# sephiroce/srf

Measured on AMD Instinct MI355X. Metric: acoustic frames/sec through SRF (123-d fbank, 3-iter DR) at 1/2/4/8 MI355X, higher is better.
Workload: dtype fp32; 1 GPU; wsj_c4: SRF L=6 PH=CH=16 DIM=32 LPAD=RPAD=2 DR iter=3, train step (fwd+bwd+allreduce+Adam); utterances_per_gpu=28, frames_per_utterance=800, global_batch=28, parallelism=dp1, launch=hipgraph (fwd+CTC+bwd)

## Files before the change

### srf_amd/csrc/cnnfe.hip

```cpp
#include <algorithm>
#include <type_traits>
#include <cmath>
#include <cstdlib>

#include "srf_common.h"
#include "srf_reduce.h"
#include "srf_rng.h"
#include "../../include/srf.h"

namespace {

constexpr int C = 64;
constexpr float kBnEps = 1e-3f;
constexpr float kBnMomentum = 0.99f;

struct Dims {
  int B, T, Fin;
  int T1, F1, T2, F2;
  int pt1, pf1, pt2, pf2;
};

inline int same_out(int n) { return (n + 1) / 2; }
inline int same_pad_before(int n) {
  const int out = same_out(n);
// ... 784 lines not shown
      return;
    } else {
    cbf8 a1, a2, a3;
    {
      float v[8];
#pragma unroll
      for (int q = 0; q < 8; ++q) v[q] = aok ? (q < 4 ? av[0][q] : av[1][q - 4]) : 0.f;
      split8v(v, a1, a2, a3);
    }
#pragma unroll
    for (int nt = 0; nt < 2; ++nt) {
      const int nrow = 32 * nt + r;
      const cbf8 b1 = *reinterpret_cast<const cbf8*>(&Bs[buf][0][nrow * kC2BStride + 8 * h]);
      const cbf8 b2 = *reinterpret_cast<const cbf8*>(&Bs[buf][1][nrow * kC2BStride + 8 * h]);
      const cbf8 b3 = *reinterpret_cast<const cbf8*>(&Bs[buf][2][nrow * kC2BStride + 8 * h]);
      cf16 cc = acc[nt];
      cc = mfma32bf(a3, b1, cc);
      cc = mfma32bf(a1, b3, cc);
      cc = mfma32bf(a2, b2, cc);
      cc = mfma32bf(a2, b1, cc);
      cc = mfma32bf(a1, b2, cc);
      cc = mfma32bf(a1, b1, cc);
      acc[nt] = cc;
    }
    }
  };
  V8 bvA[NBL], bvB[NBL];
  f4 avA[2], avB[2];
  bool okA, okB;
  load_b(0, bvA);
  load_a(0, avA, okA);
  load_b(1, bvB);
  load_a(1, avB, okB);
  store_b(0, bvA);
  __syncthreads();
  for (int kk = 0; kk < nkb; kk += 2) {
    {
      const f4 a0[2] = {avA[0], avA[1]};
      const bool ok0 = okA;
      if (kk + 2 < nkb) {
        load_b(kk + 2, bvA);
        load_a(kk + 2, avA, okA);
      }
      compute(0, a0, ok0);
      store_b(1, bvB);
      __syncthreads();
    }
    {
      const f4 a1v[2] = {avB[0], avB[1]};
      const bool ok1 = okB;
      if (kk + 3 < nkb) {
        load_b(kk + 3, bvB);
        load_a(kk + 3, avB, okB);
      }
      compute(1, a1v, ok1);
      if (kk + 2 < nkb) store_b(0, bvA);
      __syncthreads();
    }
  }
  float osc[2] = {1.f, 1.f};
  if constexpr (H) {
    osc[0] = inv_sa * wdsc[r];
    osc[1] = inv_sa * wdsc[32 + r];
  }
#pragma unroll
  for (int q = 0; q < 4; ++q)
#pragma unroll
    for (int v = 0; v < 4; ++v) {
      const int p = q0 + 32 * wv + 8 * q + 4 * h + v;
      if (p >= Pc) continue;
      const int kf = p % nkf, kt = (p / nkf) % nkt, b = p / (nkf * nkt);
      float* dst = g_x1 + (((size_t)b * d.T1 + qt + 2 * kt) * d.F1 + qf + 2 * kf) * C + r;
      dst[0] = H ? acc[0][4 * q + v] * osc[0] : acc[0][4 * q + v];
      dst[32] = H ? acc[1][4 * q + v] * osc[1] : acc[1][4 * q + v];
    }
}

constexpr int kWgChunk = 32;

struct WgDiv {
  FastDiv f2, t2;
};

constexpr int kTpPx = 64;
template <bool H>
__global__ __launch_bounds__(256) void gab_split_t_kernel(const float* __restrict__ g_ab, int P2, int P2p,
                                                          void* __restrict__ gsTv, const float* __restrict__ gmax,
                                                          int ngmax) {
  __shared__ float tile[kTpPx][2 * C + 1];
  const int tid = threadIdx.x;
  const int p0 = blockIdx.x * kTpPx;
  float sa = 1.f;
  if constexpr (H) sa = srf_exp2i(gab_exp(gmax, ngmax));
  for (int k = tid; k < kTpPx * (2 * C / 4); k += 256) {
    const int px = k / (2 * C / 4), q = k % (2 * C / 4);
    const int p = p0 + px;
    const f4 v = p < P2 ? *reinterpret_cast<const f4*>(g_ab + (size_t)p * 2 * C + 4 * q) : f4{0.f, 0.f, 0.f, 0.f};
    tile[px][4 * q] = v.x;
    tile[px][4 * q + 1] = v.y;
    tile[px][4 * q + 2] = v.z;
    tile[px][4 * q + 3] = v.w;
  }
  __syncthreads();
  const size_t plane = (size_t)2 * C * P2p;
  for (int task = tid; task < 2 * C * (kTpPx / 8); task += 256) {
    const int o = task & 7, n = task >> 3;
    float v[8];
#pragma unroll
    for (int k = 0; k < 8; ++k) v[k] = tile[8 * o + k][n];
    if constexpr (H) {
      ch8 p1, p2;
#pragma unroll
      for (int k = 0; k < 8; ++k) {
        _Float16 h1, h2;
        srf_split2h(v[k] * sa, h1, h2);
        p1[k] = h1;
        p2[k] = h2;
      }
      _Float16* dst = static_cast<_Float16*>(gsTv) + (size_t)n * P2p + p0 + 8 * o;
      *reinterpret_cast<ch8*>(dst) = p1;
      *reinterpret_cast<ch8*>(dst + plane) = p2;
    } else {
      cbf8 p1, p2, p3;
      split8v(v, p1, p2, p3);
      __bf16* dst = static_cast<__bf16*>(gsTv) + (size_t)n * P2p + p0 + 8 * o;
      *reinterpret_cast<cbf8*>(dst) = p1;
      *reinterpret_cast<cbf8*>(dst + plane) = p2;
      *reinterpret_cast<cbf8*>(dst + 2 * plane) = p3;
    }
  }
}

constexpr int kW2Chunk = 32;
constexpr int kW2AStride = 96;

typedef short ws4 __attribute__((ext_vector_type(4)));

template <typename BT>
__device__ __forceinline__ ws4 lds_tr16(const BT* p) {
  return __builtin_amdgcn_ds_read_tr16_b64_v4i16(
      (__attribute__((address_space(3))) ws4*)(reinterpret_cast<uintptr_t>(p)));
}

template <bool H>
__global__ __launch_bounds__(256) __attribute__((amdgpu_waves_per_eu(2))) void conv2_wgrad32_kernel(
    const float* __restrict__ y1, const float* __restrict__ stats1, const int* __restrict__ inp_len,
    const void* __restrict__ gsTv, int P2p, Dims d, WgDiv dv, int nsplit, int split_len, float* __restrict__ part,
    const float* __restrict__ gmax, int ngmax) {
  using BT = std::conditional_t<H, _Float16, __bf16>;
  using V8 = std::conditional_t<H, ch8, cbf8>;
  constexpr int NPL = H ? 2 : 3;
  const BT* __restrict__ gsT3 = static_cast<const BT*>(gsTv);
  __shared__ __attribute__((aligned(16))) BT As[2][NPL][kW2Chunk * kW2AStride];
  float out_sc = 1.f;
  if constexpr (H) out_sc = stats1[4 * C + 1] * srf_exp2i(-gab_exp(gmax, ngmax));
  const int tid = threadIdx.x, lane = tid & 63, wv = tid >> 6;
  const int r = lane & 31, h = lane >> 5;
  const int xcd = blockIdx.x & 7, loc = blockIdx.x >> 3;
  const int tap = loc % 9, sp = xcd + 8 * (loc / 9);
  const int dt = tap / 3, df = tap - dt * 3;
  const int P2 = d.B * d.T2 * d.F2;
  const int pbeg = sp * split_len, pend = min(P2, pbeg + split_len);
  const int px = tid >> 3, oc = tid & 7;
  float scale[8], shift[8];
  const float bsc = H ? stats1[4 * C] : 1.f;
#pragma unroll
  for (int k = 0; k < 8; ++k) {
    scale[k] = stats1[2 * C + 8 * oc + k] * bsc;
    shift[k] = stats1[3 * C + 8 * oc + k] * bsc;
  }
  f4 xv[2];
  bool xok = false;
  auto gather = [&](int pc0) {
    const int p = pc0 + px;
    const unsigned pcl = (unsigned)min(p, P2 - 1);
    const unsigned r1 = fdiv(pcl, dv.f2);
    const int f2 = (int)(pcl - r1 * d.F2);
    const unsigned bq = fdiv(r1, dv.t2);
    const int t2 = (int)(r1 - bq * d.T2), b = (int)bq;
    const int t1 = 2 * t2 - d.pt2 + dt, f1 = 2 * f2 - d.pf2 + df;
    xok = p < pend && t1 >= 0 && t1 < d.T1 && f1 >= 0 && f1 < d.F1 && t1 < ceil_div_len(inp_len[b], 2);
    const int t1c = min(max(t1, 0), d.T1 - 1), f1c = min(max(f1, 0), d.F1 - 1);
    const float* src = y1 + (((size_t)b * d.T1 + t1c) * d.F1 + f1c) * C + 8 * oc;
    xv[0] = *reinterpret_cast<const f4*>(src);
    xv[1] = *reinterpret_cast<const f4*>(src + 4);
  };
  auto put = [&](int buf) {
    float v[8];
#pragma unroll
    for (int k = 0; k < 8; ++k) v[k] = xok ? (k < 4 ? xv[0][k] : xv[1][k - 4]) * scale[k] + shift[k] : 0.f;
    const int o = px * kW2AStride + 8 * oc;
    if constexpr (H) {
      ch8 p1, p2;
#pragma unroll
      for (int k = 0; k < 8; ++k) {
        _Float16 h1, h2;
        srf_split2h(v[k], h1, h2);
        p1[k] = h1;
        p2[k] = h2;
      }
      *reinterpret_cast<ch8*>(&As[buf][0][o]) = p1;
      *reinterpret_cast<ch8*>(&As[buf][1][o]) = p2;
    } else {
      cbf8 p1, p2, p3;
      split8v(v, p1, p2, p3);
      *reinterpret_cast<cbf8*>(&As[buf][0][o]) = p1;
      *reinterpret_cast<cbf8*>(&As[buf][1][o]) = p2;
      *reinterpret_cast<cbf8*>(&As[buf][2][o]) = p3;
    }
  };
  const int gg = lane >> 4, qq = (lane >> 2) & 3, pp = lane & 3;
  const int a_off = (8 * (gg >> 1) + qq) * kW2AStride + 16 * (gg & 1) + 4 * pp;
  auto read_a = [&](const BT* img, int kb, int mt) {
    const BT* base = img + a_off + 16 * kb * kW2AStride + 32 * mt;
    const ws4 lo = lds_tr16(base), hi = lds_tr16(base + 4 * kW2AStride);
    return __builtin_bit_cast(V8, __builtin_shufflevector(lo, hi, 0, 1, 2, 3, 4, 5, 6, 7));
  };
  const size_t bplane = (size_t)2 * C * P2p;
  const BT* brow = gsT3 + (size_t)(32 * wv + r) * P2p + 8 * h;
  V8 bc[2][NPL], bn[2][NPL];
  auto load_bf = [&](int pc0, V8 (&bf)[2][NPL]) {
#pragma unroll
    for (int kb = 0; kb < 2; ++kb)
#pragma unroll
      for (int pl = 0; pl < NPL; ++pl) bf[kb][pl] = *reinterpret_cast<const V8*>(brow + pl * bplane + pc0 + 16 * kb);
  };

  cf16 acc[2];
  acc[0] = cf16{};
  acc[1] = cf16{};
  const int nch = (pend - pbeg + kW2Chunk - 1) / kW2Chunk;
  if (nch > 0) {
    gather(pbeg);
    load_bf(pbeg, bc);
    put(0);
  }
  __syncthreads();
  for (int ch = 0; ch < nch; ++ch) {
    const bool more = ch + 1 < nch;
    const int buf = ch & 1;
    if (more) {
      gather(pbeg + (ch + 1) * kW2Chunk);
      load_bf(pbeg + (ch + 1) * kW2Chunk, bn);
    }
#pragma unroll
    for (int kb = 0; kb < 2; ++kb)
#pragma unroll
      for (int mt = 0; mt < 2; ++mt) {
        if constexpr (H) {
          const ch8 a1 = read_a(As[buf][0], kb, mt);
          const ch8 a2 = read_a(As[buf][1], kb, mt);
          cf16 cc = acc[mt];
          cc = mfma32h(a2, bc[kb][0], cc);
          cc = mfma32h(a1, bc[kb][1], cc);
          cc = mfma32h(a1, bc[kb][0], cc);
          acc[mt] = cc;
        } else {
          const cbf8 a1 = read_a(As[buf][0], kb, mt);
          const cbf8 a2 = read_a(As[buf][1], kb, mt);
          const cbf8 a3 = read_a(As[buf][2], kb, mt);
          cf16 cc = acc[mt];
          cc = mfma32bf(a3, bc[kb][0], cc);
          cc = mfma32bf(a1, bc[kb][2], cc);
          cc = mfma32bf(a2, bc[kb][1], cc);
          cc = mfma32bf(a2, bc[kb][0], cc);
          cc = mfma32bf(a1, bc[kb][1], cc);
          cc = mfma32bf(a1, bc[kb][0], cc);
          acc[mt] = cc;
        }
      }
    if (more) {
      put(buf ^ 1);
#pragma unroll
      for (int kb = 0; kb < 2; ++kb)
#pragma unroll
        for (int pl = 0; pl < NPL; ++pl) bc[kb][pl] = bn[kb][pl];
    }
    __syncthreads();
  }
  float* dst = part + ((size_t)sp * 9 + tap) * C * 2 * C + 32 * wv + r;
#pragma unroll
  for (int mt = 0; mt < 2; ++mt)
#pragma unroll
    for (int q = 0; q < 4; ++q)
#pragma unroll
      for (int v = 0; v < 4; ++v) dst[(size_t)(32 * mt + 8 * q + 4 * h + v) * 2 * C] = acc[mt][4 * q + v] * out_sc;
}

__global__ void conv2_wgrad_reduce_kernel(const float* __restrict__ part, int nsplit, float* __restrict__ gka,
                                          float* __restrict__ gkb) {
  const int idx = blockIdx.x * blockDim.x + threadIdx.x;
  if (idx >= 9 * C * 2 * C) return;
  float s = 0.f;
#pragma unroll 8
  for (int k = 0; k < nsplit; ++k) s += part[(size_t)k * 9 * C * 2 * C + idx];
  const int n = idx % (2 * C);
  const int tc = idx / (2 * C);
  if (n < C)
    gka[(size_t)tc * C + n] = s;
  else
    gkb[(size_t)tc * C + n - C] = s;
}

__global__ __launch_bounds__(256) void conv1_bwd_kernel(
    const float* __restrict__ feats, const int* __restrict__ inp_len, Dims d, const float* __restrict__ g_x1,
    const float* __restrict__ y1, const unsigned char* __restrict__ sel1, const float* __restrict__ stats1,
    const float* __restrict__ gamma1, const float* __restrict__ bnsum1, float drop_p, unsigned long long seed, const unsigned long long* __restrict__ seed_src,
    float* __restrict__ part) {
  seed = srf_step_seed(seed, seed_src);
  extern __shared__ __attribute__((aligned(16))) float win[];
  __shared__ float sh[kRows1][20][C];
  const int c = threadIdx.x & (C - 1);
  const int w = __builtin_amdgcn_readfirstlane(threadIdx.x >> 6);
  const int P = d.B * d.T1 * d.F1;
  const float mean = stats1[c], rstd = stats1[C + c], gam = gamma1[c];
  const float sdy_n = bnsum1[c] / (float)P, sdyxh_n = bnsum1[C + c] / (float)P;
  const float keep_scale = 1.f / (1.f - drop_p);
  float acc[20];
#pragma unroll
  for (int j = 0; j < 20; ++j) acc[j] = 0.f;
  const Tile1 tl = stage_rows1(feats, d, win);
  const int t1 = tl.t1_0 + w;
  if (t1 < d.T1) {
    const float mask = t1 < ceil_div_len(inp_len[tl.b], 2) ? 1.f : 0.f;
    const int pbase = (tl.b * d.T1 + t1) * d.F1;
    constexpr int FB = 8;
    for (int f0 = 0; f0 < d.F1; f0 += FB) {
      float gxv[FB], yv[FB];
      unsigned char sv[FB];
#pragma unroll
      for (int u = 0; u < FB; ++u) {
        const int o = (pbase + min(f0 + u, d.F1 - 1)) * C + c;
        gxv[u] = g_x1[o];
        yv[u] = y1[o];
        sv[u] = sel1[o];
      }
#pragma unroll
      for (int u = 0; u < FB; ++u) {
        const int f1 = f0 + u;
        if (f1 >= d.F1) break;
        const int o = (pbase + f1) * C + c;
        const float gy = bn_bwd_elem(gxv[u], yv[u], mask, mean, rstd, gam, sdy_n, sdyxh_n);
        const bool sl = sv[u] != 0;
        float ga = sl ? gy : 0.f, gb = sl ? 0.f : gy;
        if (drop_p > 0.f) {
          bool ka, kb;
          srf_keep2(seed, kStreamConv0a, o, drop_p, ka, kb);
          ga *= ka ? keep_scale : 0.f;
          gb *= kb ? keep_scale : 0.f;
        }
        float x[9];
        window9_lds(win, tl, d, w, f1, x);
        acc[18] += ga;
        acc[19] += gb;
#pragma unroll
        for (int k = 0; k < 9; ++k) {
          acc[k] += x[k] * ga;
          acc[9 + k] += x[k] * gb;
        }
      }
    }
  }
#pragma unroll
  for (int j = 0; j < 20; ++j) sh[w][j][c] = acc[j];
  __syncthreads();
  for (int j = w; j < 20; j += kRows1) {
    float v = 0.f;
#pragma unroll
    for (int r = 0; r < kRows1; ++r) v += sh[r][j][c];
    part[((size_t)blockIdx.x * 20 + j) * C + c] = v;
  }
}

inline int conv1_blocks(const Dims& d) { return d.B * ((d.T1 + kRows1 - 1) / kRows1); }
inline size_t conv1_lds(const Dims& d) { return (size_t)(2 * kRows1 + 1) * (d.Fin + 2) * sizeof(float); }

struct FwdSaved {
  float *y1, *y2, *stats1, *stats2;
  unsigned char *sel1, *sel2;
  size_t bytes;
};

FwdSaved saved_layout(const Dims& d, void* base) {
  const size_t P1 = (size_t)d.B * d.T1 * d.F1, P2 = (size_t)d.B * d.T2 * d.F2;
  size_t off = 0;
  auto take = [&](size_t bytes) {
    size_t o = off;
    off += srf::align_up(bytes, 256);
    return o;
  };
  const size_t oy1 = take(P1 * C * 4), oy2 = take(P2 * C * 4), os1 = take(5 * C * 4), os2 = take(5 * C * 4),
               osel1 = take(P1 * C), osel2 = take(P2 * C);
  char* b = static_cast<char*>(base);
  FwdSaved s;
  s.y1 = (float*)(b + oy1);
  s.y2 = (float*)(b + oy2);
  s.stats1 = (float*)(b + os1);
  s.stats2 = (float*)(b + os2);
  s.sel1 = (unsigned char*)(b + osel1);
  s.sel2 = (unsigned char*)(b + osel2);
  s.bytes = off;
  return s;
}

constexpr int kBnMerge = 32;

int bn_finalize(const float* part, int nparts, float* merged, const float* gamma, const float* beta, float* mmean,
                float* mvar, int training, float* stats, hipStream_t st, const float* ymax = nullptr,
                int nymax = 0) {
  const int per = (nparts + kBnMerge - 1) / kBnMerge;
  hipLaunchKernelGGL(bn_merge_kernel, dim3(kBnMerge), dim3(256), 0, st, part, nparts, per, merged);
  SRF_LAUNCH_CHECK("bn_merge");
  hipLaunchKernelGGL(bn_finalize_kernel, dim3(1), dim3(1024), 0, st, merged, kBnMerge, gamma, beta, mmean, mvar,
                     training, stats, ymax, nymax);
  SRF_LAUNCH_CHECK("bn_finalize");
  return SRF_OK;
}

struct FwdWs {
  float *part1, *part2, *wp, *merged;
  _Float16* wp2;
  float* wsc;
  float* ymax;
  size_t bytes;
};

FwdWs fwd_ws_layout(const Dims& d, void* base) {
  const size_t P2 = (size_t)d.B * d.T2 * d.F2;
  const size_t nb2 = (P2 + 63) / 64;
  size_t off = 0;
  auto take = [&](size_t bytes) {
    size_t o = off;
    off += srf::align_up(bytes, 256);
    return o;
  };
  const size_t op1 = take((size_t)conv1_blocks(d) * 3 * C * 4), op2 = take(nb2 * 3 * C * 4),
               owp = take((size_t)9 * 2 * C * C * 4), omg = take((size_t)kBnMerge * 3 * C * 4),
               owp2 = take((size_t)2 * 9 * 2 * C * C * 2), owsc = take((size_t)2 * C * 4),
               oym = take((size_t)conv1_blocks(d) * 4);
  char* b = static_cast<char*>(base);
  FwdWs w;
  w.wp2 = (_Float16*)(b + owp2);
  w.wsc = (float*)(b + owsc);
  w.ymax = (float*)(b + oym);
  w.merged = (float*)(b + omg);
  w.part1 = (float*)(b + op1);
  w.part2 = (float*)(b + op2);
  w.wp = (float*)(b + owp);
  w.bytes = off;
  return w;
}

int check_dims(int B, int T, int Fin, int nfilt) {
  SRF_REQUIRE(B > 0 && T > 0 && Fin > 0, "bad CNN-FE shape B=%d T=%d F=%d", B, T, Fin);
  SRF_REQUIRE(nfilt == C, "model-conv-filter-num must be %d (got %d)", C, nfilt);
  return SRF_OK;
}

}

extern "C" {

int srf_cnnfe_out_dims(int T, int feat_dim, int* T2, int* F2) {
  SRF_REQUIRE(T > 0 && feat_dim > 0 && T2 && F2, "bad arguments");
  Dims d = make_dims(1, T, feat_dim);
  *T2 = d.T2;
  *F2 = d.F2;
  return SRF_OK;
}

size_t srf_cnnfe_saved_bytes(int B, int T, int feat_dim, int nfilt) {
  (void)nfilt;
  return saved_layout(make_dims(B, T, feat_dim), nullptr).bytes;
}

size_t srf_cnnfe_fwd_workspace(int B, int T, int feat_dim, int nfilt) {
  (void)nfilt;
  return fwd_ws_layout(make_dims(B, T, feat_dim), nullptr).bytes;
}

int srf_cnnfe_fwd(const float* feats, const int* inp_len, int B, int T, int feat_dim, int nfilt,
                  const float* k0a, const float* b0a, const float* k0b, const float* b0b, const float* gamma0,
                  const float* beta0, const float* k1a, const float* b1a, const float* k1b, const float* b1b,
                  const float* gamma1, const float* beta1, float* mmean0, float* mvar0, float* mmean1, float* mvar1,
                  int training, float drop_p, unsigned long long seed, float* out, void* saved, size_t saved_bytes,
                  void* workspace, size_t workspace_bytes, void* stream) {
  int rc = check_dims(B, T, feat_dim, nfilt);
  if (rc) return rc;
  SRF_REQUIRE(feats && inp_len && k0a && b0a && k0b && b0b && gamma0 && beta0 && k1a && b1a && k1b && b1b &&
                  gamma1 && beta1 && mmean0 && mvar0 && mmean1 && mvar1 && out && saved && workspace,
              "null pointer argument");
  SRF_REQUIRE(drop_p >= 0.f && drop_p < 1.f, "dropout rate %f out of [0,1)", drop_p);
  const Dims d = make_dims(B, T, feat_dim);
  FwdSaved sv = saved_layout(d, saved);
  FwdWs w = fwd_ws_layout(d, workspace);
  if (saved_bytes < sv.bytes || workspace_bytes < w.bytes) {
    srf::set_error("CNN-FE buffers too small (saved %zu < %zu or workspace %zu < %zu)", saved_bytes, sv.bytes,
                   workspace_bytes, w.bytes);
    return SRF_EWORKSPACE;
  }
  hipStream_t st = static_cast<hipStream_t>(stream);
  const size_t P2 = (size_t)d.B * d.T2 * d.F2;
  const int nb2 = (int)((P2 + 63) / 64);
  int nparts2 = nb2;
  const int npack = (kPackW2Threads + 64 * kRows1 - 1) / (64 * kRows1);
  hipLaunchKernelGGL(conv1_fwd_kernel, dim3(conv1_blocks(d) + npack), dim3(64 * kRows1), conv1_lds(d), st, feats,
                     inp_len, d, k0a, b0a, k0b, b0b, training, drop_p, seed, srf::seed_source(), sv.y1, sv.sel1,
                     w.part1, conv1_blocks(d), k1a, k1b, w.wp2, w.wsc, w.ymax);
  SRF_LAUNCH_CHECK("conv1_fwd");
  if ((rc = bn_finalize(w.part1, conv1_blocks(d), w.merged, gamma0, beta0, mmean0, mvar0, training, sv.stats1, st,
                        w.ymax, conv1_blocks(d))))
    return rc;
  SRF_LAUNCH_CHECK("bn_finalize(1)");
  {
    const int nb32 = (int)((P2 + kC2Px - 1) / kC2Px);
    hipLaunchKernelGGL(conv2_fwd32_kernel, dim3(nb32), dim3(64 * kC2Waves), 0, st, sv.y1, sv.stats1, inp_len, d,
                       w.wp2, w.wsc, b1a, b1b, training, drop_p, seed, srf::seed_source(), sv.y2, sv.sel2,
                       w.part2);
    SRF_LAUNCH_CHECK("conv2_fwd32");
    nparts2 = nb32;
  }
  if ((rc = bn_finalize(w.part2, nparts2, w.merged, gamma1, beta1, mmean1, mvar1, training, sv.stats2, st)))
    return rc;
  SRF_LAUNCH_CHECK("bn_finalize(2)");
  hipLaunchKernelGGL(bn_apply_kernel, dim3(1024), dim3(256), 0, st, sv.y2, sv.stats2, inp_len, d.B, d.T2, d.F2, 4,
                     out);
  SRF_LAUNCH_CHECK("bn_apply");
  return SRF_OK;
}

}

namespace {
struct BwdWs2 {
  float *bnpart, *bnsum2, *bnsum1, *g_ab, *biaspart, *g_x1, *wq, *wpart, *c1part, *c1sum, *scratch;
  __bf16* gsT3;
  float* gmax;
  float* wdsc;
  int P2p;
  size_t bytes;
};

constexpr int kBnBlocks = 1024;
constexpr int kWgrad32SplitsMax = 128;
constexpr int kWgrad32Splits = 56;

BwdWs2 bwd_ws_layout(const Dims& d, void* base) {
  const size_t P1 = (size_t)d.B * d.T1 * d.F1, P2 = (size_t)d.B * d.T2 * d.F2;
  size_t off = 0;
  auto take = [&](size_t bytes) {
    size_t o = off;
    off += srf::align_up(bytes, 256);
    return o;
  };
  const size_t obp = take((size_t)kBnBlocks * 2 * C * 4), os2 = take(2 * C * 4), os1 = take(2 * C * 4),
               oab = take(P2 * 2 * C * 4), obias = take((size_t)kBnBlocks * 2 * C * 4), ogx = take(P1 * C * 4),
               owq = take((size_t)9 * 2 * C * C * 4), owp = take((size_t)kWgrad32SplitsMax * 9 * C * 2 * C * 4),
               oc1 = take((size_t)conv1_blocks(d) * 20 * C * 4), oc1s = take(20 * C * 4),
               oscr = take(srf::colsum_scratch_floats(std::max(conv1_blocks(d), kBnBlocks), 20 * C) * 4);
  const int P2p = (int)((P2 + kTpPx - 1) / kTpPx * kTpPx);
  const size_t ogs3 = take((size_t)3 * 2 * C * P2p * 2);
  const size_t ogm = take((size_t)kBnBlocks * 4), ods = take((size_t)C * 4);
  char* b = static_cast<char*>(base);
  BwdWs2 w;
  w.bnpart = (float*)(b + obp);
  w.bnsum2 = (float*)(b + os2);
  w.bnsum1 = (float*)(b + os1);
  w.g_ab = (float*)(b + oab);
  w.biaspart = (float*)(b + obias);
  w.g_x1 = (float*)(b + ogx);
  w.wq = (float*)(b + owq);
  w.wpart = (float*)(b + owp);
  w.c1part = (float*)(b + oc1);
  w.c1sum = (float*)(b + oc1s);
  w.scratch = (float*)(b + oscr);
  w.gsT3 = (__bf16*)(b + ogs3);
  w.gmax = (float*)(b + ogm);
  w.wdsc = (float*)(b + ods);
  w.P2p = P2p;
  w.bytes = off;
  return w;
}

}

extern "C" {

size_t srf_cnnfe_bwd_workspace(int B, int T, int feat_dim, int nfilt) {
  (void)nfilt;
  return bwd_ws_layout(make_dims(B, T, feat_dim), nullptr).bytes;
}

int srf_cnnfe_bwd(const float* feats, const int* inp_len, int B, int T, int feat_dim, int nfilt, const float* gamma0,
                  const float* k1a, const float* k1b, const float* gamma1, float drop_p, unsigned long long seed,
                  const void* saved, const float* g_out, float* g_k0a, float* g_b0a, float* g_k0b, float* g_b0b,
                  float* g_gamma0, float* g_beta0, float* g_k1a, float* g_b1a, float* g_k1b, float* g_b1b,
                  float* g_gamma1, float* g_beta1, void* workspace, size_t workspace_bytes, void* stream) {
  return srf_cnnfe_bwd_parts(SRF_CNNFE_BWD_ALL, feats, inp_len, B, T, feat_dim, nfilt, gamma0, k1a, k1b, gamma1, drop_p,
                             seed, saved, g_out, g_k0a, g_b0a, g_k0b, g_b0b, g_gamma0, g_beta0, g_k1a, g_b1a, g_k1b,
                             g_b1b, g_gamma1, g_beta1, workspace, workspace_bytes, stream);
}

int srf_cnnfe_bwd_parts(int parts, const float* feats, const int* inp_len, int B, int T, int feat_dim, int nfilt,
                        const float* gamma0, const float* k1a, const float* k1b, const float* gamma1, float drop_p,
                        unsigned long long seed, const void* saved, const float* g_out, float* g_k0a, float* g_b0a,
                        float* g_k0b, float* g_b0b, float* g_gamma0, float* g_beta0, float* g_k1a, float* g_b1a,
                        float* g_k1b, float* g_b1b, float* g_gamma1, float* g_beta1, void* workspace,
                        size_t workspace_bytes, void* stream) {
  SRF_REQUIRE(parts > 0 && (parts & ~SRF_CNNFE_BWD_ALL) == 0, "CNN-FE backward: bad parts mask %d", parts);
  int rc = check_dims(B, T, feat_dim, nfilt);
  if (rc) return rc;
  SRF_REQUIRE(feats && inp_len && gamma0 && k1a && k1b && gamma1 && saved && g_out && g_k0a && g_b0a && g_k0b &&
                  g_b0b && g_gamma0 && g_beta0 && g_k1a && g_b1a && g_k1b && g_b1b && g_gamma1 && g_beta1 &&
                  workspace,
              "null pointer argument");
  SRF_REQUIRE(((uintptr_t)g_out & 15) == 0 && ((uintptr_t)saved & 255) == 0 && ((uintptr_t)workspace & 255) == 0,
              "CNN-FE backward: g_out must be 16-byte and saved / workspace 256-byte aligned");
  const Dims d = make_dims(B, T, feat_dim);
  FwdSaved sv = saved_layout(d, const_cast<void*>(saved));
  BwdWs2 w = bwd_ws_layout(d, workspace);
  if (workspace_bytes < w.bytes) {
    srf::set_error("CNN-FE backward workspace too small: %zu < %zu", workspace_bytes, w.bytes);
    return SRF_EWORKSPACE;
  }
  hipStream_t st = static_cast<hipStream_t>(stream);
  const int P2 = d.B * d.T2 * d.F2;
  __bf16* wq3 = reinterpret_cast<__bf16*>(w.wq);
  _Float16* wq2h = reinterpret_cast<_Float16*>(w.wq);
  if (parts & SRF_CNNFE_BWD_PREP) {
  hipLaunchKernelGGL(bn_bwd_reduce_kernel, dim3(kBnBlocks), dim3(256), 0, st, g_out, sv.y2, sv.stats2, inp_len, d.B,
                     d.T2, d.F2, 4, w.bnpart);
  SRF_LAUNCH_CHECK("bn_bwd_reduce(2)");
  if ((rc = srf::colsum(w.bnpart, kBnBlocks, 2 * C, w.bnsum2, w.scratch, st, srf::ColSplit{{g_beta1, g_gamma1, nullptr, nullptr}, {C, C, 0, 0}})))
    return rc;
  const int npack = (kPackW2tF16Threads + 255) / 256;
  hipLaunchKernelGGL(conv2_bwd_prep_kernel, dim3(kBnBlocks + npack), dim3(256), 0, st, g_out, sv.y2, sv.sel2,
                     sv.stats2, gamma1, w.bnsum2, inp_len, d, drop_p, seed, srf::seed_source(), w.g_ab, w.biaspart,
                     kBnBlocks, k1a, k1b, wq3, wq2h, w.wdsc, w.gmax);
  SRF_LAUNCH_CHECK("conv2_bwd_prep");
  if ((rc = srf::colsum(w.biaspart, kBnBlocks, 2 * C, nullptr, w.scratch, st, srf::ColSplit{{g_b1a, g_b1b, nullptr, nullptr}, {C, C, 0, 0}})))
    return rc;
  }
  if (parts & SRF_CNNFE_BWD_DATA) {
    DgCls cls{};
    for (int c = 0; c < 4; ++c) {
      const int qt = c >> 1, qf = c & 1;
      const int Pc = d.B * ((d.T1 - qt + 1) / 2) * ((d.F1 - qf + 1) / 2);
      cls.boff[c + 1] = cls.boff[c] + (Pc + kD2Px - 1) / kD2Px;
    }
    hipLaunchKernelGGL(conv2_dgrad32_kernel<true>, dim3(cls.boff[4]), dim3(64 * kD2Waves), 0, st, w.g_ab,
                       (const void*)wq2h, d, cls, w.g_x1, (const float*)w.gmax, kBnBlocks, (const float*)w.wdsc);
    SRF_LAUNCH_CHECK("conv2_dgrad32");
  }
  const WgDiv dv{make_fastdiv(d.F2), make_fastdiv(d.T2)};
  const int nsplit = kWgrad32Splits;
  if (parts & SRF_CNNFE_BWD_WGRAD) {
    static_assert(kW2Chunk == kWgChunk, "wgrad splits are whole chunks");
    const int split_len = ((P2 + nsplit - 1) / nsplit + kWgChunk - 1) / kWgChunk * kWgChunk;
    hipLaunchKernelGGL(gab_split_t_kernel<true>, dim3(w.P2p / kTpPx), dim3(256), 0, st, w.g_ab, P2, w.P2p,
                       (void*)w.gsT3, (const float*)w.gmax, kBnBlocks);
    SRF_LAUNCH_CHECK("gab_split_t");
    hipLaunchKernelGGL(conv2_wgrad32_kernel<true>, dim3(9 * nsplit), dim3(256), 0, st, sv.y1, sv.stats1, inp_len,
                       (const void*)w.gsT3, w.P2p, d, dv, nsplit, split_len, w.wpart, (const float*)w.gmax,
                       kBnBlocks);
    SRF_LAUNCH_CHECK("conv2_wgrad32");
    hipLaunchKernelGGL(conv2_wgrad_reduce_kernel, dim3((9 * C * 2 * C + 255) / 256), dim3(256), 0, st, w.wpart,
                       nsplit, g_k1a, g_k1b);
    SRF_LAUNCH_CHECK("conv2_wgrad_reduce");
  }
  if (!(parts & SRF_CNNFE_BWD_DATA)) return SRF_OK;
  hipLaunchKernelGGL(bn_bwd_reduce_kernel, dim3(kBnBlocks), dim3(256), 0, st, w.g_x1, sv.y1, sv.stats1, inp_len, d.B,
                     d.T1, d.F1, 2, w.bnpart);
  SRF_LAUNCH_CHECK("bn_bwd_reduce(1)");
  if ((rc = srf::colsum(w.bnpart, kBnBlocks, 2 * C, w.bnsum1, w.scratch, st, srf::ColSplit{{g_beta0, g_gamma0, nullptr, nullptr}, {C, C, 0, 0}})))
    return rc;
  hipLaunchKernelGGL(conv1_bwd_kernel, dim3(conv1_blocks(d)), dim3(64 * kRows1), conv1_lds(d), st, feats, inp_len, d, w.g_x1, sv.y1,
                     sv.sel1, sv.stats1, gamma0, w.bnsum1, drop_p, seed, srf::seed_source(), w.c1part);
  SRF_LAUNCH_CHECK("conv1_bwd");
  if ((rc = srf::colsum(w.c1part, conv1_blocks(d), 20 * C, nullptr, w.scratch, st,
                        srf::ColSplit{{g_k0a, g_k0b, g_b0a, g_b0b, nullptr, nullptr}, {9 * C, 9 * C, C, C, 0, 0}})))
    return rc;
  return SRF_OK;
}

}
```

Before: 3.035 million frames/s.

## Compute conv2 weight gradient by time rows with fused fp16-split staging

Adds a row-range conv2 weight-gradient kernel for F2<=32. Each block streams output time rows, normalises y1 and scales g_ab in registers, splits them into fp16 hi/lo pairs in LDS, and runs three MFMAs per tap. The input rows are kept in a four-slot ring so the overlapping time tap is reused. This removes the separate gab_split_t transpose pass and its bf16 workspace. The trade-off is 256 partial slabs, which need a wider reduction kernel and more workspace, and a different fp16-split precision path.

```diff
diff --git a/srf_amd/csrc/cnnfe.hip b/srf_amd/csrc/cnnfe.hip
--- a/srf_amd/csrc/cnnfe.hip
+++ b/srf_amd/csrc/cnnfe.hip
@@ -1110,6 +1110,186 @@
     gkb[(size_t)tc * C + n - C] = s;
 }
 
+#ifndef SRF_CONV2_WGRAD_ROWS
+#define SRF_CONV2_WGRAD_ROWS 1
+#endif
+
+constexpr int kWrRanges = 256;
+constexpr int kWrCh = 32;
+constexpr int kWrSub = 33 * kWrCh;
+constexpr int kWrSlot = 4 * kWrSub;
+constexpr int kWrBStride = 160;
+constexpr int kWrBPlane = 32 * kWrBStride;
+
+__global__ __launch_bounds__(256) __attribute__((amdgpu_waves_per_eu(2))) void conv2_wgrad_rows_kernel(
+    const float* __restrict__ y1, const float* __restrict__ stats1, const int* __restrict__ inp_len,
+    const float* __restrict__ g_ab, Dims d, int rows_per, float* __restrict__ part, const float* __restrict__ gmax,
+    int ngmax) {
+  __shared__ __attribute__((aligned(16))) _Float16 As[4 * kWrSlot];
+  __shared__ __attribute__((aligned(16))) _Float16 Bs[2 * kWrBPlane];
+  const int tid = threadIdx.x, lane = tid & 63, wv = tid >> 6;
+  const int r = lane & 31, h = lane >> 5;
+  const int hc = (blockIdx.x >> 3) & 1, rg = (blockIdx.x & 7) + 8 * (blockIdx.x >> 4);
+  const int R = d.B * d.T2;
+  const int rbeg = (int)min((long long)R, (long long)rg * rows_per), rend = min(R, rbeg + rows_per);
+  for (int k = tid; k < 4 * kWrSlot / 8; k += 256) *reinterpret_cast<ch8*>(&As[8 * k]) = ch8{};
+  for (int k = tid; k < 2 * kWrBPlane / 8; k += 256) *reinterpret_cast<ch8*>(&Bs[8 * k]) = ch8{};
+  const int ea = gab_exp(gmax, ngmax);
+  const float sa = srf_exp2i(ea);
+  const float out_sc = stats1[4 * C + 1] * srf_exp2i(-ea);
+  __syncthreads();
+
+  const int ac = tid >> 2, aoc = tid & 3;
+  const int af1 = ac - d.pf2;
+  const bool acol_ok = af1 >= 0 && af1 < d.F1;
+  const int af1c = min(max(af1, 0), d.F1 - 1);
+  const int a_lds = (ac & 1) * 2 * kWrSub + (ac >> 1) * kWrCh + 8 * aoc;
+  const int bpx = tid >> 4, bo = tid & 15;
+  float scale[8], shift[8];
+  const float bsc = stats1[4 * C];
+#pragma unroll
+  for (int k = 0; k < 8; ++k) {
+    scale[k] = stats1[2 * C + 32 * hc + 8 * aoc + k] * bsc;
+    shift[k] = stats1[3 * C + 32 * hc + 8 * aoc + k] * bsc;
+  }
+  f4 xv[3][2], gv[2][2];
+  bool xok[3] = {false, false, false};
+  auto load_row = [&](int b, int t2, bool fresh) {
+    const int alen1 = ceil_div_len(inp_len[b], 2);
+#pragma unroll
+    for (int dt = 0; dt < 3; ++dt) {
+      if (dt == 0 && !fresh) continue;
+      const int t1 = 2 * t2 - d.pt2 + dt;
+      xok[dt] = acol_ok && t1 >= 0 && t1 < d.T1 && t1 < alen1;
+      const int t1c = min(max(t1, 0), d.T1 - 1);
+      const float* src = y1 + (((size_t)b * d.T1 + t1c) * d.F1 + af1c) * C + 32 * hc + 8 * aoc;
+      xv[dt][0] = *reinterpret_cast<const f4*>(src);
+      xv[dt][1] = *reinterpret_cast<const f4*>(src + 4);
+    }
+#pragma unroll
+    for (int u = 0; u < 2; ++u) {
+      const int pxc = min(bpx + 16 * u, d.F2 - 1);
+      const float* src = g_ab + (((size_t)b * d.T2 + t2) * d.F2 + pxc) * 2 * C + 8 * bo;
+      gv[u][0] = *reinterpret_cast<const f4*>(src);
+      gv[u][1] = *reinterpret_cast<const f4*>(src + 4);
+    }
+  };
+  auto put_row = [&](int t2, bool fresh) {
+#pragma unroll
+    for (int dt = 0; dt < 3; ++dt) {
+      if (dt == 0 && !fresh) continue;
+      ch8 p1, p2;
+#pragma unroll
+      for (int k = 0; k < 8; ++k) {
+        const float v = xok[dt] ? (k < 4 ? xv[dt][0][k] : xv[dt][1][k - 4]) * scale[k] + shift[k] : 0.f;
+        _Float16 h1, h2;
+        srf_split2h(v, h1, h2);
+        p1[k] = h1;
+        p2[k] = h2;
+      }
+      _Float16* dst = As + ((2 * t2 + dt) & 3) * kWrSlot + a_lds;
+      *reinterpret_cast<ch8*>(dst) = p1;
+      *reinterpret_cast<ch8*>(dst + kWrSub) = p2;
+    }
+#pragma unroll
+    for (int u = 0; u < 2; ++u) {
+      const int px = bpx + 16 * u;
+      const bool ok = px < d.F2;
+      ch8 p1, p2;
+#pragma unroll
+      for (int k = 0; k < 8; ++k) {
+        const float v = ok ? (k < 4 ? gv[u][0][k] : gv[u][1][k - 4]) * sa : 0.f;
+        _Float16 h1, h2;
+        srf_split2h(v, h1, h2);
+        p1[k] = h1;
+        p2[k] = h2;
+      }
+      _Float16* dst = Bs + px * kWrBStride + 8 * bo;
+      *reinterpret_cast<ch8*>(dst) = p1;
+      *reinterpret_cast<ch8*>(dst + kWrBPlane) = p2;
+    }
+  };
+  const int gg = lane >> 4, qq = (lane >> 2) & 3, pp = lane & 3;
+  const int a_off = (8 * (gg >> 1) + qq) * kWrCh + 16 * (gg & 1) + 4 * pp;
+  const int b_off = (8 * (gg >> 1) + qq) * kWrBStride + 32 * wv + 16 * (gg & 1) + 4 * pp;
+  auto tr8 = [&](const _Float16* base, int stride) {
+    const ws4 lo = lds_tr16(base), hi = lds_tr16(base + 4 * stride);
+    return __builtin_bit_cast(ch8, __builtin_shufflevector(lo, hi, 0, 1, 2, 3, 4, 5, 6, 7));
+  };
+  cf16 acc[9];
+#pragma unroll
+  for (int tap = 0; tap < 9; ++tap) acc[tap] = cf16{};
+  auto compute = [&](int t2) {
+#pragma unroll
+    for (int kb = 0; kb < 2; ++kb) {
+      const ch8 b1 = tr8(Bs + b_off + 16 * kb * kWrBStride, kWrBStride);
+      const ch8 b2 = tr8(Bs + kWrBPlane + b_off + 16 * kb * kWrBStride, kWrBStride);
+#pragma unroll
+      for (int tap = 0; tap < 9; ++tap) {
+        const int dt = tap / 3, df = tap - dt * 3;
+        const _Float16* img =
+            As + ((2 * t2 + dt) & 3) * kWrSlot + (df & 1) * 2 * kWrSub + ((df >> 1) + 16 * kb) * kWrCh + a_off;
+        const ch8 a1 = tr8(img, kWrCh);
+        const ch8 a2 = tr8(img + kWrSub, kWrCh);
+        cf16 cc = acc[tap];
+        cc = mfma32h(a2, b1, cc);
+        cc = mfma32h(a1, b2, cc);
+        cc = mfma32h(a1, b1, cc);
+        acc[tap] = cc;
+      }
+    }
+  };
+
+  int b = rbeg / d.T2, t2 = rbeg - b * d.T2;
+  if (rbeg < rend) {
+    load_row(b, t2, true);
+    put_row(t2, true);
+  }
+  __syncthreads();
+  for (int row = rbeg; row < rend; ++row) {
+    const bool more = row + 1 < rend;
+    const bool nfresh = t2 + 1 == d.T2;
+    const int nb = nfresh ? b + 1 : b, nt2 = nfresh ? 0 : t2 + 1;
+    if (more) load_row(nb, nt2, nfresh);
+    compute(t2);
+    __syncthreads();
+    if (more) put_row(nt2, nfresh);
+    __syncthreads();
+    b = nb;
+    t2 = nt2;
+  }
+  float* dst = part + ((size_t)rg * 9 * C + 32 * hc) * 2 * C + 32 * wv + r;
+#pragma unroll
+  for (int tap = 0; tap < 9; ++tap)
+#pragma unroll
+    for (int q = 0; q < 4; ++q)
+#pragma unroll
+      for (int v = 0; v < 4; ++v)
+        dst[((size_t)tap * C + 8 * q + 4 * h + v) * 2 * C] = acc[tap][4 * q + v] * out_sc;
+}
+
+__global__ __launch_bounds__(256) void conv2_wgrad_reduce_rows_kernel(const float* __restrict__ part,
+                                                                      float* __restrict__ gka,
+                                                                      float* __restrict__ gkb) {
+  static_assert(kWrRanges == 256 && (9 * C * 2 * C) % 128 == 0, "eight groups of 32 slabs");
+  __shared__ f4 sums[8][32];
+  const int j = threadIdx.x & 31, g = threadIdx.x >> 5;
+  const size_t idx = (size_t)blockIdx.x * 128 + 4 * j;
+  const float* src = part + (size_t)g * 9 * C * 2 * C + idx;
+  f4 s = {0.f, 0.f, 0.f, 0.f};
+#pragma unroll 8
+  for (int k = 0; k < 32; ++k) s += *reinterpret_cast<const f4*>(src + (size_t)8 * k * 9 * C * 2 * C);
+  sums[g][j] = s;
+  __syncthreads();
+  if (g != 0) return;
+  for (int k = 1; k < 8; ++k) s += sums[k][j];
+  const int n = (int)(idx % (2 * C));
+  const size_t tc = idx / (2 * C);
+  float* dst = n < C ? gka + tc * C + n : gkb + tc * C + n - C;
+#pragma unroll
+  for (int k = 0; k < 4; ++k) dst[k] = s[k];
+}
+
 __global__ __launch_bounds__(256) void conv1_bwd_kernel(
     const float* __restrict__ feats, const int* __restrict__ inp_len, Dims d, const float* __restrict__ g_x1,
     const float* __restrict__ y1, const unsigned char* __restrict__ sel1, const float* __restrict__ stats1,
@@ -1352,6 +1532,7 @@
 constexpr int kBnBlocks = 1024;
 constexpr int kWgrad32SplitsMax = 128;
 constexpr int kWgrad32Splits = 56;
+inline bool wgrad_by_rows(const Dims& d) { return SRF_CONV2_WGRAD_ROWS && d.F2 <= 32; }
 
 BwdWs2 bwd_ws_layout(const Dims& d, void* base) {
   const size_t P1 = (size_t)d.B * d.T1 * d.F1, P2 = (size_t)d.B * d.T2 * d.F2;
@@ -1363,11 +1544,12 @@
   };
   const size_t obp = take((size_t)kBnBlocks * 2 * C * 4), os2 = take(2 * C * 4), os1 = take(2 * C * 4),
                oab = take(P2 * 2 * C * 4), obias = take((size_t)kBnBlocks * 2 * C * 4), ogx = take(P1 * C * 4),
-               owq = take((size_t)9 * 2 * C * C * 4), owp = take((size_t)kWgrad32SplitsMax * 9 * C * 2 * C * 4),
+               owq = take((size_t)9 * 2 * C * C * 4),
+               owp = take((size_t)std::max(kWgrad32SplitsMax, kWrRanges) * 9 * C * 2 * C * 4),
                oc1 = take((size_t)conv1_blocks(d) * 20 * C * 4), oc1s = take(20 * C * 4),
                oscr = take(srf::colsum_scratch_floats(std::max(conv1_blocks(d), kBnBlocks), 20 * C) * 4);
   const int P2p = (int)((P2 + kTpPx - 1) / kTpPx * kTpPx);
-  const size_t ogs3 = take((size_t)3 * 2 * C * P2p * 2);
+  const size_t ogs3 = take(wgrad_by_rows(d) ? 0 : (size_t)3 * 2 * C * P2p * 2);
   const size_t ogm = take((size_t)kBnBlocks * 4), ods = take((size_t)C * 4);
   char* b = static_cast<char*>(base);
   BwdWs2 w;
@@ -1462,7 +1644,15 @@
   }
   const WgDiv dv{make_fastdiv(d.F2), make_fastdiv(d.T2)};
   const int nsplit = kWgrad32Splits;
-  if (parts & SRF_CNNFE_BWD_WGRAD) {
+  if ((parts & SRF_CNNFE_BWD_WGRAD) && wgrad_by_rows(d)) {
+    const int rows_per = (d.B * d.T2 + kWrRanges - 1) / kWrRanges;
+    hipLaunchKernelGGL(conv2_wgrad_rows_kernel, dim3(2 * kWrRanges), dim3(256), 0, st, sv.y1, sv.stats1, inp_len,
+                       (const float*)w.g_ab, d, rows_per, w.wpart, (const float*)w.gmax, kBnBlocks);
+    SRF_LAUNCH_CHECK("conv2_wgrad_rows");
+    hipLaunchKernelGGL(conv2_wgrad_reduce_rows_kernel, dim3(9 * C * 2 * C / 128), dim3(256), 0, st, w.wpart, g_k1a,
+                       g_k1b);
+    SRF_LAUNCH_CHECK("conv2_wgrad_reduce_rows");
+  } else if (parts & SRF_CNNFE_BWD_WGRAD) {
     static_assert(kW2Chunk == kWgChunk, "wgrad splits are whole chunks");
     const int split_len = ((P2 + nsplit - 1) / nsplit + kWgChunk - 1) / kWgChunk * kWgChunk;
     hipLaunchKernelGGL(gab_split_t_kernel<true>, dim3(w.P2p / kTpPx), dim3(256), 0, st, w.g_ab, P2, w.P2p,
```

After: 3.092 million frames/s (median of 6 runs). 1.02x the previous value.
